# jeffreyyu0602/quantized-training

Hardware: AMD Instinct MI355X
Metric: quantized_elements_per_sec (higher is better)
Workload: dtype bf16; 1 GPU; llama-2-7b-shaped LLaMA (32 layers, hidden 4096, random init) WikiText-style window eval B=1 S=1024 stride 512, fake-quant activation=e4m3 weight=e4m3, --quantize_forward gemm (weights re-quantized every forward); route=eager, parallelism=dp1 (windows round-robin, metric all_gather only), launch=hipGraph replay, valid=True

## Files before the change

### quantized-training_amd/csrc/qt_model_ops.hip

```cpp
#include <hip/hip_runtime.h>
#include <stdint.h>

#include "../../include/qt_hip.h"
#include "qt_device.h"
#include "qt_dispatch.h"
#include "qt_formats.h"
#include "qt_value_codes.h"
#include "qt_value_rows.h"

namespace {

constexpr int kNormThreads = 256;
constexpr int kNormMaxVec = 8;

struct NormExtra {
    uint2 *y8[2];
    qt_format fmt[2];
    int e5m2[2];
};

template <int FQ, bool ADD = false, int EXTRA = 0, int NV = kNormMaxVec>
__global__ __launch_bounds__(kNormThreads) void rmsnorm_kernel(const uint4 *__restrict__ x, const uint4 *__restrict__ w,
                                                               uint4 *__restrict__ y, int nvec, float inv_cols, float eps,
                                                               uint2 *__restrict__ y8, qt_format fmt,
// ... 118 lines not shown
            const float g0 = bf_lo(p[j]), g1 = bf_hi(p[j]);
            const float s0 = bf16_round(g0 / (1.0f + expf(-g0))), s1 = bf16_round(g1 / (1.0f + expf(-g1)));
            pr[j] = pack_bf16x2(s0 * bf_lo(q[j]), s1 * bf_hi(q[j]));
        }
        fq_rows_words<4, false>(pr, o, rnd);
        y[i] = uint4{o[0], o[1], o[2], o[3]};
    }
}

template <bool E5M2>
__global__ __launch_bounds__(256) void silu_mul_fq8_kernel(const uint4 *__restrict__ g, const uint4 *__restrict__ u,
                                                           uint4 *__restrict__ y, uint2 *__restrict__ y8, size_t nvec,
                                                           qt_format fmt, size_t cv, size_t rs_g, size_t rs_u) {
    for (size_t i = (size_t)blockIdx.x * 256 + threadIdx.x; i < nvec; i += (size_t)gridDim.x * 256) {
        const size_t row = i / cv, col = i - row * cv;
        const uint4 a = g[row * rs_g + col], b = u[row * rs_u + col];
        const uint32_t p[4] = {a.x, a.y, a.z, a.w}, q[4] = {b.x, b.y, b.z, b.w};
        uint32_t o[4];
#pragma unroll
        for (int j = 0; j < 4; ++j) {
            const float g0 = bf_lo(p[j]), g1 = bf_hi(p[j]);
            const float s0 = bf16_round(g0 / (1.0f + expf(-g0))), s1 = bf16_round(g1 / (1.0f + expf(-g1)));
            o[j] = pack_bf16x2(s0 * bf_lo(q[j]), s1 * bf_hi(q[j]));
        }
        const uint2 codes = fq8_hw_vec8<E5M2>(o, fmt);
        y[i] = uint4{o[0], o[1], o[2], o[3]};
        y8[i] = codes;
    }
}

struct RopeArgs {
    const uint16_t *x;
    uint16_t *y;
    const uint16_t *cos, *sin;
    long B, S, H, D;
    size_t nvec;
    long rsv;
};

__device__ __forceinline__ void rope_one(const RopeArgs &a, size_t i) {
    const long dv = a.D / 8;
    const long d8 = (long)(i % dv);
    const size_t bsh = i / dv;
    const size_t bs = bsh / (size_t)a.H;
    const long half = dv / 2;
    const bool low = d8 < half;
    const size_t in_row = bs * (size_t)a.rsv + (bsh % (size_t)a.H) * dv;
    const uint4 xv = *(const uint4 *)(a.x + (in_row + d8) * 8);
    const uint4 pv = *(const uint4 *)(a.x + (in_row + (low ? d8 + half : d8 - half)) * 8);
    const uint4 cv = *(const uint4 *)(a.cos + (bs * dv + d8) * 8);
    const uint4 sv = *(const uint4 *)(a.sin + (bs * dv + d8) * 8);
    const uint32_t X[4] = {xv.x, xv.y, xv.z, xv.w}, P[4] = {pv.x, pv.y, pv.z, pv.w};
    const uint32_t C[4] = {cv.x, cv.y, cv.z, cv.w}, S[4] = {sv.x, sv.y, sv.z, sv.w};
    const float sgn = low ? -1.0f : 1.0f;
    uint32_t o[4];
#pragma unroll
    for (int j = 0; j < 4; ++j) {
        const float a0 = bf16_round(bf_lo(X[j]) * bf_lo(C[j])), a1 = bf16_round(bf_hi(X[j]) * bf_hi(C[j]));
        const float b0 = bf16_round(sgn * bf_lo(P[j]) * bf_lo(S[j])), b1 = bf16_round(sgn * bf_hi(P[j]) * bf_hi(S[j]));
        o[j] = pack_bf16x2(a0 + b0, a1 + b1);
    }
    *(uint4 *)(a.y + i * 8) = uint4{o[0], o[1], o[2], o[3]};
}

__global__ __launch_bounds__(256) void rope_kernel(RopeArgs q, RopeArgs k) {
    const size_t total = q.nvec + k.nvec;
    for (size_t i = (size_t)blockIdx.x * 256 + threadIdx.x; i < total; i += (size_t)gridDim.x * 256) {
        if (i < q.nvec) rope_one(q, i);
        else rope_one(k, i - q.nvec);
    }
}

struct RopeFqArgs {
    RopeArgs r;
    qt_format fmt;
    uint8_t *y8;
    int e5m2;
    int inner;
    qt_format inner_fmt;
    const uint16_t *map;
    const uint16_t *rows_lds;
};

template <bool CODES = false>
__device__ __forceinline__ void rope_fq_token(const RopeFqArgs &a, size_t bs0, uint32_t tpb, size_t tokens) {
    const uint32_t dv = (uint32_t)a.r.D / 8, half = dv / 2, nv = (uint32_t)a.r.H * dv;
    const uint32_t S = (uint32_t)a.r.S;
    for (uint32_t i = threadIdx.x; i < tpb * nv; i += 256) {
        const uint32_t lt = tpb == 1 ? 0u : i / nv, v = i - lt * nv;
        const size_t bs = bs0 + lt;
        if (bs >= tokens) break;
        const uint32_t b = (uint32_t)(bs / S), s = (uint32_t)(bs - (size_t)b * S);
        const uint16_t *xrow = a.r.x + bs * (size_t)a.r.rsv * 8;
        const uint16_t *crow = a.r.cos + bs * dv * 8, *srow = a.r.sin + bs * dv * 8;
        const uint32_t h = v / dv, d8 = v - h * dv;
        const bool low = d8 < half;
        const uint4 xv = *(const uint4 *)(xrow + (size_t)v * 8);
        uint32_t out[4] = {xv.x, xv.y, xv.z, xv.w};
        if (a.r.cos) {
            const uint4 pv = *(const uint4 *)(xrow + (size_t)(low ? v + half : v - half) * 8);
            const uint4 cv = *(const uint4 *)(crow + d8 * 8);
            const uint4 sv = *(const uint4 *)(srow + d8 * 8);
            const uint32_t X[4] = {xv.x, xv.y, xv.z, xv.w}, P[4] = {pv.x, pv.y, pv.z, pv.w};
            const uint32_t C[4] = {cv.x, cv.y, cv.z, cv.w}, S[4] = {sv.x, sv.y, sv.z, sv.w};
            const float sgn = low ? -1.0f : 1.0f;
#pragma unroll
            for (int j = 0; j < 4; ++j) {
                float a0 = bf16_round(bf_lo(X[j]) * bf_lo(C[j])), a1 = bf16_round(bf_hi(X[j]) * bf_hi(C[j]));
                if (!CODES && a.inner) {
                    if (a.map) {
                        const Rounder<kFmtRows> rin{a.fmt, a.rows_lds, a.map};
                        a0 = qt_u2f(rin(qt_f2u(a0)));
                        a1 = qt_u2f(rin(qt_f2u(a1)));
                    } else {
                        a0 = qt_u2f(qt_fp_sat_u32(qt_f2u(a0), a.inner_fmt.p0, a.inner_fmt.p1, a.inner_fmt.fhi));
                        a1 = qt_u2f(qt_fp_sat_u32(qt_f2u(a1), a.inner_fmt.p0, a.inner_fmt.p1, a.inner_fmt.fhi));
                    }
                }
                const float b0 = bf16_round(sgn * bf_lo(P[j]) * bf_lo(S[j])), b1 = bf16_round(sgn * bf_hi(P[j]) * bf_hi(S[j]));
                out[j] = pack_bf16x2(a0 + b0, a1 + b1);
            }
        }
        const size_t o = (((size_t)b * (size_t)a.r.H + h) * (size_t)a.r.S + s) * dv + d8;
        if (CODES || a.y8) {
            const uint2 codes = a.e5m2 ? fq8_hw_vec8<true>(out, a.fmt) : fq8_hw_vec8<false>(out, a.fmt);
            *(uint2 *)(a.y8 + o * 8) = codes;
        } else if (a.map) {
            const Rounder<kFmtRows> rnd{a.fmt, a.rows_lds, a.map};
            const uint32_t oin[4] = {out[0], out[1], out[2], out[3]};
            fq_rows_words<4, false>(oin, out, rnd);
        } else {
#pragma unroll
            for (int j = 0; j < 4; ++j) {
                const uint32_t r0 = qt_fp_sat_u32(out[j] << 16, a.fmt.p0, a.fmt.p1, a.fmt.fhi);
                const uint32_t r1 = qt_fp_sat_u32(out[j] & 0xFFFF0000u, a.fmt.p0, a.fmt.p1, a.fmt.fhi);
                out[j] = (r0 >> 16) | (r1 & 0xFFFF0000u);
            }
        }
        if (a.r.y) *(uint4 *)(a.r.y + o * 8) = uint4{out[0], out[1], out[2], out[3]};
    }
}

__global__ __launch_bounds__(256) void rope_fq_kernel(RopeFqArgs q, RopeFqArgs k, unsigned tpb) {
    __shared__ uint4 s_rope_rows[512];
    if (q.map) {
        const uint4 *gr = (const uint4 *)(q.map + QT_MAP_ENTRIES);
        const int nrows = (q.fmt.p1 & 2) ? 512 : 256;
        for (int i = threadIdx.x; i < nrows; i += 256) s_rope_rows[i] = gr[i];
        __syncthreads();
        q.rows_lds = k.rows_lds = (const uint16_t *)s_rope_rows;
    }
    const size_t tokens = (size_t)q.r.B * (size_t)q.r.S;
    for (size_t bs = (size_t)blockIdx.x * tpb; bs < tokens; bs += (size_t)gridDim.x * tpb) {
        rope_fq_token(q, bs, tpb, tokens);
        rope_fq_token(k, bs, tpb, tokens);
    }
}

struct ValueArgs {
    const uint16_t *v;
    uint8_t *vt8;
    long sb, sh, sk, Sk;
    int H, nkb;
    qt_format fmt;
};

template <bool VE5M2, int VD, bool CODES = false>
__global__ __launch_bounds__(256) void rope_fq_value_kernel(RopeFqArgs q, RopeFqArgs k, ValueArgs v, unsigned rope_blocks, unsigned tpb) {
    __shared__ __attribute__((aligned(16))) uint8_t tile[VD * 128];
    if (blockIdx.x < rope_blocks) {
        const size_t tokens = (size_t)q.r.B * (size_t)q.r.S;
        for (size_t bs = (size_t)blockIdx.x * tpb; bs < tokens; bs += (size_t)rope_blocks * tpb) {
            rope_fq_token<CODES>(q, bs, tpb, tokens);
            rope_fq_token<CODES>(k, bs, tpb, tokens);
        }
    } else {
        const unsigned vb = blockIdx.x - rope_blocks;
        value_codes_block<VE5M2, VD>(tile, v.v, v.vt8, (int)(vb % (unsigned)v.nkb), (long)(vb / (unsigned)v.nkb), v.H, v.Sk, v.sb, v.sh, v.sk, v.fmt);
    }
}

struct ValueRowsArgs {
    const uint16_t *v;
    uint16_t *vt;
    long sb, sh, sk, Sk;
    int H, nkb;
};
struct WeightPassArgs {
    const uint4 *w;
    uint4 *wq;
    size_t nvec;
    unsigned blocks;
};

__global__ __launch_bounds__(256) void rope_map_value_kernel(RopeFqArgs q, RopeFqArgs k, ValueRowsArgs v, WeightPassArgs wp, unsigned rope_blocks,
                                                             unsigned tpb) {
    __shared__ __attribute__((aligned(16))) uint16_t tile[value_rows_tile_elems<64>()];
    __shared__ uint4 s_rows[512];
    {
        const uint4 *gr = (const uint4 *)(q.map + QT_MAP_ENTRIES);
        const int nrows = (q.fmt.p1 & 2) ? 512 : 256;
        for (int i = threadIdx.x; i < nrows; i += 256) s_rows[i] = gr[i];
        __syncthreads();
        q.rows_lds = k.rows_lds = (const uint16_t *)s_rows;
    }
    if (blockIdx.x < wp.blocks) {
        const Rounder<kFmtRows> rnd{q.fmt, (const uint16_t *)s_rows, q.map};
        constexpr int kU = 4;
        const size_t stride = (size_t)wp.blocks * 256;
        for (size_t i0 = (size_t)blockIdx.x * 256 + threadIdx.x; i0 < wp.nvec; i0 += stride * kU) {
            uint4 a[kU];
#pragma unroll
            for (int u = 0; u < kU; ++u)
                if (i0 + u * stride < wp.nvec) a[u] = wp.w[i0 + u * stride];
#pragma unroll
            for (int u = 0; u < kU; ++u) {
                if (i0 + u * stride < wp.nvec) {
                    const uint32_t in[4] = {a[u].x, a[u].y, a[u].z, a[u].w};
                    uint32_t o[4];
                    fq_rows_words<4, false>(in, o, rnd);
                    wp.wq[i0 + u * stride] = uint4{o[0], o[1], o[2], o[3]};
                }
            }
        }
        return;
    }
    const unsigned bid = blockIdx.x - wp.blocks;
    if (bid < rope_blocks) {
        const size_t tokens = (size_t)q.r.B * (size_t)q.r.S;
        for (size_t bs = (size_t)bid * tpb; bs < tokens; bs += (size_t)rope_blocks * tpb) {
            rope_fq_token(q, bs, tpb, tokens);
            rope_fq_token(k, bs, tpb, tokens);
        }
    } else {
        const unsigned vb = bid - rope_blocks;
        const Rounder<kFmtRows> rnd{q.fmt, (const uint16_t *)s_rows, q.map};
        value_t_rows_block<64>(tile, rnd, v.v, v.vt, v.H, v.Sk, v.sb, v.sh, v.sk, (long)(vb / (unsigned)v.nkb), (int)(vb % (unsigned)v.nkb), (int)threadIdx.x);
    }
}

struct LnArgs {
    const uint4 *x, *res, *w, *b;
    uint4 *y, *yq;
    uint2 *y8;
    long rows;
    int nvec;
    float inv_cols, eps;
    qt_format fmt;
    int n_extra;
    NormExtra extra;
};

template <int G, int FQ, bool ADD, int NV = kNormMaxVec>
__global__ __launch_bounds__(256) void layernorm_kernel(LnArgs a) {
    constexpr int RPB = 256 / G;
    __shared__ float s_part[2][4];
    const int sub = threadIdx.x / G, lane = threadIdx.x % G;
    const long row = (long)blockIdx.x * RPB + sub;
    if (G == 64 && row >= a.rows) return;
    const size_t base = (size_t)row * (size_t)a.nvec;
    uint4 v[NV];
    float sum = 0.0f;
#pragma unroll
    for (int i = 0; i < NV; ++i) {
        const int c = lane + i * G;
        if (c < a.nvec) {
            v[i] = a.x[base + c];
            if constexpr (ADD) {
                const uint4 r = a.res[base + c];
                v[i].x = pack_bf16x2(bf_lo(v[i].x) + bf_lo(r.x), bf_hi(v[i].x) + bf_hi(r.x));
                v[i].y = pack_bf16x2(bf_lo(v[i].y) + bf_lo(r.y), bf_hi(v[i].y) + bf_hi(r.y));
                v[i].z = pack_bf16x2(bf_lo(v[i].z) + bf_lo(r.z), bf_hi(v[i].z) + bf_hi(r.z));
                v[i].w = pack_bf16x2(bf_lo(v[i].w) + bf_lo(r.w), bf_hi(v[i].w) + bf_hi(r.w));
            }
            sum += (bf_lo(v[i].x) + bf_hi(v[i].x)) + (bf_lo(v[i].y) + bf_hi(v[i].y)) + (bf_lo(v[i].z) + bf_hi(v[i].z)) +
                   (bf_lo(v[i].w) + bf_hi(v[i].w));
        }
    }
    auto reduce = [&](float t, int slot) {
#pragma unroll
        for (int off = 32; off >= 1; off >>= 1) t += __shfl_xor(t, off, 64);
        if constexpr (G == 256) {
            if ((threadIdx.x & 63) == 0) s_part[slot][threadIdx.x >> 6] = t;
            __syncthreads();
            t = (s_part[slot][0] + s_part[slot][1]) + (s_part[slot][2] + s_part[slot][3]);
        }
        return t;
    };
    const float mean = reduce(sum, 0) * a.inv_cols;
    float sq = 0.0f;
#pragma unroll
    for (int i = 0; i < NV; ++i) {
        const int c = lane + i * G;
        if (c < a.nvec) {
            const uint32_t q[4] = {v[i].x, v[i].y, v[i].z, v[i].w};
#pragma unroll
            for (int j = 0; j < 4; ++j) {
                const float d0 = bf_lo(q[j]) - mean, d1 = bf_hi(q[j]) - mean;
                sq += d0 * d0;
                sq += d1 * d1;
            }
        }
    }
    const float rstd = rsqrtf(reduce(sq, 1) * a.inv_cols + a.eps);
#pragma unroll
    for (int i = 0; i < NV; ++i) {
        const int c = lane + i * G;
        if (c < a.nvec) {
            const uint4 ww = a.w[c], bb = a.b[c];
            const uint32_t q[4] = {v[i].x, v[i].y, v[i].z, v[i].w}, g[4] = {ww.x, ww.y, ww.z, ww.w}, h[4] = {bb.x, bb.y, bb.z, bb.w};
            uint32_t o[4];
#pragma unroll
            for (int j = 0; j < 4; ++j)
                o[j] = pack_bf16x2(bf_lo(g[j]) * (rstd * (bf_lo(q[j]) - mean)) + bf_lo(h[j]),
                                   bf_hi(g[j]) * (rstd * (bf_hi(q[j]) - mean)) + bf_hi(h[j]));
// ... 313 lines not shown
}

static int launch_layernorm_any(const LnArgs &a, int fq, bool with_residual, void *stream) {
    hipStream_t st = (hipStream_t)stream;
    const long rows = a.rows;
    const bool residual = with_residual;
    if (a.nvec <= 128) {
        const unsigned blocks = (unsigned)((rows + 3) / 4);
        if (residual) launch_layernorm<64, true>(a, fq, blocks, st);
        else launch_layernorm<64, false>(a, fq, blocks, st);
    } else {
        if (residual) launch_layernorm<256, true>(a, fq, (unsigned)rows, st);
        else launch_layernorm<256, false>(a, fq, (unsigned)rows, st);
    }
    return qt_launch_status();
}

int qt_gelu_bf16(const uint16_t *x, uint16_t *y, uint8_t *y8, size_t n, const qt_format *fmt, void *stream) {
    if (n == 0) return QT_OK;
    if (!x || (!y && !y8)) return QT_ERR_BAD_ARG;
    const int fq = y8 ? qt_fp8_code(fmt) : 0;
    if (y8 && !fq) return QT_ERR_BAD_ARG;
    if ((n & 7) || (((uintptr_t)x | (uintptr_t)y) & 15u) || ((uintptr_t)y8 & 7u)) return QT_ERR_UNALIGNED;
    const size_t nvec = n / 8;
    size_t blocks = (nvec + 255) / 256;
    if (blocks > 256 * 32) blocks = 256 * 32;
    hipStream_t st = (hipStream_t)stream;
    const qt_format f = fq ? *fmt : qt_format{};
    qt_pick<0, 1, 2>(fq, [&](auto FQ) {
        gelu_kernel<decltype(FQ)::value><<<(unsigned)blocks, 256, 0, st>>>((const uint4 *)x, (uint4 *)y, (uint2 *)y8, nvec, f);
    });
    return qt_launch_status();
}

int qt_silu_mul_bf16(const uint16_t *gate, const uint16_t *up, uint16_t *y, size_t rows, size_t cols, size_t gate_row_stride,
                     size_t up_row_stride, void *stream) {
    const size_t n = rows * cols;
    if (n == 0) return QT_OK;
    if (!gate || !up || !y || gate_row_stride < cols || up_row_stride < cols) return QT_ERR_BAD_ARG;
    if ((cols & 7) || ((gate_row_stride | up_row_stride) & 7) || (((uintptr_t)gate | (uintptr_t)up | (uintptr_t)y) & 15u))
        return QT_ERR_UNALIGNED;
    const size_t nvec = n / 8;
    size_t blocks = (nvec + 255) / 256;
    if (blocks > 256 * 32) blocks = 256 * 32;
    silu_mul_kernel<<<(unsigned)blocks, 256, 0, (hipStream_t)stream>>>((const uint4 *)gate, (const uint4 *)up, (uint4 *)y, nvec,
                                                                       cols / 8, gate_row_stride / 8, up_row_stride / 8);
    return qt_launch_status();
}

int qt_silu_mul_fq8_bf16(const uint16_t *gate, const uint16_t *up, uint16_t *y, uint8_t *y8, size_t rows, size_t cols,
                         size_t gate_row_stride, size_t up_row_stride, const qt_format *fmt, void *stream) {
    const size_t n = rows * cols;
    if (n == 0) return QT_OK;
    const int f8 = qt_fp8_code(fmt);
    if (!gate || !up || !y || !y8 || !f8 || gate_row_stride < cols || up_row_stride < cols) return QT_ERR_BAD_ARG;
    if ((cols & 7) || ((gate_row_stride | up_row_stride) & 7) || (((uintptr_t)gate | (uintptr_t)up | (uintptr_t)y) & 15u) ||
        ((uintptr_t)y8 & 7u))
        return QT_ERR_UNALIGNED;
    const size_t nvec = n / 8;
    size_t blocks = (nvec + 255) / 256;
    if (blocks > 256 * 32) blocks = 256 * 32;
    qt_pick_bool(f8 == 2, [&](auto E5M2) {
        silu_mul_fq8_kernel<decltype(E5M2)::value><<<(unsigned)blocks, 256, 0, (hipStream_t)stream>>>((const uint4 *)gate, (const uint4 *)up, (uint4 *)y, (uint2 *)y8, nvec,
                                                                                                      *fmt, cols / 8, gate_row_stride / 8, up_row_stride / 8);
    });
    return qt_launch_status();
}

int qt_rope_bf16(const uint16_t *q, const uint16_t *k, const uint16_t *cos, const uint16_t *sin, uint16_t *q_out,
                 uint16_t *k_out, long B, long S, long Hq, long Hk, long D, long q_row_stride, long k_row_stride, void *stream) {
    if (B * S * D == 0) return QT_OK;
    if (!q || !k || !cos || !sin || !q_out || !k_out || B < 0 || S < 0 || Hq < 0 || Hk < 0) return QT_ERR_BAD_ARG;
    if (D % 16 || (((uintptr_t)q | (uintptr_t)k | (uintptr_t)cos | (uintptr_t)sin | (uintptr_t)q_out | (uintptr_t)k_out) & 15u))
        return QT_ERR_UNALIGNED;
    if (q_row_stride < Hq * D || k_row_stride < Hk * D || (q_row_stride | k_row_stride) % 8) return QT_ERR_BAD_ARG;
    RopeArgs aq{q, q_out, cos, sin, B, S, Hq, D, (size_t)(B * S * Hq * D / 8), q_row_stride / 8};
    RopeArgs ak{k, k_out, cos, sin, B, S, Hk, D, (size_t)(B * S * Hk * D / 8), k_row_stride / 8};
    size_t blocks = (aq.nvec + ak.nvec + 255) / 256;
    if (blocks > 256 * 32) blocks = 256 * 32;
    rope_kernel<<<(unsigned)blocks, 256, 0, (hipStream_t)stream>>>(aq, ak);
    return qt_launch_status();
}

static int rope_fq_launch(const uint16_t *q, const uint16_t *k, const uint16_t *cos, const uint16_t *sin, uint16_t *q_out, uint16_t *k_out,
                          uint8_t *q_out8, uint8_t *k_out8, long B, long S, long Hq, long Hk, long D, long q_row_stride, long k_row_stride,
                          const qt_format *fmt_q, const qt_format *fmt_k, bool need_values, const uint16_t *v, uint8_t *vt8, long v_sb, long v_sh,
                          long v_sk, const qt_format *fmt_v, void *stream, const qt_format *inner_q = nullptr, const qt_format *inner_k = nullptr) {
    if (B * S * D == 0) return QT_OK;
    if ((inner_q && inner_q->kind != QT_FMT_FP_SAT) || (inner_k && inner_k->kind != QT_FMT_FP_SAT) || ((inner_q || inner_k) && !cos)) return QT_ERR_BAD_ARG;
    if (!q || !k || (need_values && !cos) || (cos == nullptr) != (sin == nullptr) || !fmt_q || !fmt_k || B < 0 || S < 0 || Hq < 0 || Hk < 0)
        return QT_ERR_BAD_ARG;
    if (need_values ? (!q_out || !k_out) : (!q_out8 || !k_out8 || (q_out == nullptr) != (k_out == nullptr))) return QT_ERR_BAD_ARG;
    if (fmt_q->kind != QT_FMT_FP_SAT || fmt_k->kind != QT_FMT_FP_SAT) return QT_ERR_BAD_ARG;
    if (D % 16 || (((uintptr_t)q | (uintptr_t)k | (uintptr_t)cos | (uintptr_t)sin | (uintptr_t)q_out | (uintptr_t)k_out) & 15u))
        return QT_ERR_UNALIGNED;
    if (q_row_stride < Hq * D || k_row_stride < Hk * D || (q_row_stride | k_row_stride) % 8) return QT_ERR_BAD_ARG;
    if (((uintptr_t)q_out8 | (uintptr_t)k_out8) & 7u) return QT_ERR_UNALIGNED;
    if ((q_out8 && !qt_fp8_code(fmt_q)) || (k_out8 && !qt_fp8_code(fmt_k))) return QT_ERR_BAD_ARG;
    RopeFqArgs aq{{q, q_out, cos, sin, B, S, Hq, D, (size_t)(B * S * Hq * D / 8), q_row_stride / 8}, *fmt_q, q_out8, qt_fp8_code(fmt_q) == 2 ? 1 : 0,
                  inner_q ? 1 : 0, inner_q ? *inner_q : qt_format{}, nullptr, nullptr};
    RopeFqArgs ak{{k, k_out, cos, sin, B, S, Hk, D, (size_t)(B * S * Hk * D / 8), k_row_stride / 8}, *fmt_k, k_out8, qt_fp8_code(fmt_k) == 2 ? 1 : 0,
                  inner_k ? 1 : 0, inner_k ? *inner_k : qt_format{}, nullptr, nullptr};
    if (Hq * D / 8 > 0xFFFFFFFFl || Hk * D / 8 > 0xFFFFFFFFl || B > 0x7FFFFFFFl || S > 0x7FFFFFFFl) return QT_ERR_BAD_ARG;
    const long nv_max = (Hq > Hk ? Hq : Hk) * D / 8;
    const unsigned tpb = nv_max >= 256 || nv_max < 1 ? 1u : (unsigned)(256 / nv_max);
    size_t blocks = ((size_t)B * (size_t)S + tpb - 1) / tpb;
    if (blocks > 256 * 64) blocks = 256 * 64;
    hipStream_t st = (hipStream_t)stream;
    if (!v) {
        rope_fq_kernel<<<(unsigned)blocks, 256, 0, st>>>(aq, ak, tpb);
        return qt_launch_status();
    }
    if (!vt8 || !qt_fp8_code(fmt_v) || (D != 64 && D != 128) || S % 128 != 0 || B * Hk > 65535) return QT_ERR_BAD_ARG;
    if ((((uintptr_t)v | (uintptr_t)vt8) & 15u) || ((v_sb | v_sh | v_sk) & 7)) return QT_ERR_UNALIGNED;
    ValueArgs av{v, vt8, v_sb, v_sh, v_sk, S, (int)Hk, (int)(S / 128), *fmt_v};
    const unsigned total = (unsigned)blocks + (unsigned)(B * Hk * (S / 128));
    const bool ve5 = qt_fp8_code(fmt_v) == 2;
    if (D == 128) {
        const bool codes = aq.y8 && ak.y8 && !aq.inner && !ak.inner && !aq.map && !ak.map;
        if (codes && !ve5) rope_fq_value_kernel<false, 128, true><<<total, 256, 0, st>>>(aq, ak, av, (unsigned)blocks, tpb);
        else if (ve5) rope_fq_value_kernel<true, 128><<<total, 256, 0, st>>>(aq, ak, av, (unsigned)blocks, tpb);
        else rope_fq_value_kernel<false, 128><<<total, 256, 0, st>>>(aq, ak, av, (unsigned)blocks, tpb);
    } else {
        const bool codes = aq.y8 && ak.y8 && !aq.inner && !ak.inner && !aq.map && !ak.map;
        if (codes && !ve5) rope_fq_value_kernel<false, 64, true><<<total, 256, 0, st>>>(aq, ak, av, (unsigned)blocks, tpb);
        else if (ve5) rope_fq_value_kernel<true, 64><<<total, 256, 0, st>>>(aq, ak, av, (unsigned)blocks, tpb);
        else rope_fq_value_kernel<false, 64><<<total, 256, 0, st>>>(aq, ak, av, (unsigned)blocks, tpb);
    }
    return qt_launch_status();
}

int qt_rope_fq_bf16(const uint16_t *q, const uint16_t *k, const uint16_t *cos, const uint16_t *sin, uint16_t *q_out,
                    uint16_t *k_out, uint8_t *q_out8, uint8_t *k_out8, long B, long S, long Hq, long Hk, long D,
                    long q_row_stride, long k_row_stride, const qt_format *fmt_q, const qt_format *fmt_k, void *stream) {
    return rope_fq_launch(q, k, cos, sin, q_out, k_out, q_out8, k_out8, B, S, Hq, Hk, D, q_row_stride, k_row_stride, fmt_q, fmt_k, true, nullptr,
                          nullptr, 0, 0, 0, nullptr, stream);
}

int qt_rope_fq_value(const uint16_t *q, const uint16_t *k, const uint16_t *cos, const uint16_t *sin, uint16_t *q_out, uint16_t *k_out,
                     uint8_t *q_out8, uint8_t *k_out8, long B, long S, long Hq, long Hk, long D, long q_row_stride, long k_row_stride,
                     const qt_format *fmt_q, const qt_format *fmt_k, const uint16_t *v, uint8_t *vt8, long v_stride_b, long v_stride_h,
                     long v_stride_k, const qt_format *fmt_v, void *stream) {
    return rope_fq_launch(q, k, cos, sin, q_out, k_out, q_out8, k_out8, B, S, Hq, Hk, D, q_row_stride, k_row_stride, fmt_q, fmt_k, false, v, vt8,
                          v_stride_b, v_stride_h, v_stride_k, fmt_v, stream);
}

static bool map_format_ok(const qt_format *fmt, const uint16_t *map) {
    return fmt && map && fmt->kind == QT_FMT_LUT && (fmt->p1 & 1) && (((uintptr_t)map) & 15u) == 0;
}

int qt_rmsnorm_map_bf16(const uint16_t *x, const uint16_t *residual, const uint16_t *weight, uint16_t *sum, uint16_t *y, long rows, long cols,
                        float eps, const qt_format *fmt, const uint16_t *map, int quantize_sum, void *stream) {
    if (rows * cols == 0) return QT_OK;
    if (!x || !weight || !y || rows < 0 || cols < 0 || (residual != nullptr) != (sum != nullptr) || !map_format_ok(fmt, map)) return QT_ERR_BAD_ARG;
    if (cols % 8 || cols > (long)kNormThreads * kNormMaxVec * 8 ||
        (((uintptr_t)x | (uintptr_t)residual | (uintptr_t)weight | (uintptr_t)sum | (uintptr_t)y) & 15u))
        return QT_ERR_UNALIGNED;
    hipStream_t st = (hipStream_t)stream;
    const int nvec = (int)(cols / 8);
    const float inv = 1.0f / (float)cols;
    if (residual) launch_rms<3, true, 0>((unsigned)rows, nvec, st, (const uint4 *)x, (const uint4 *)weight, (uint4 *)y, nvec, inv, eps, nullptr, *fmt, (const uint4 *)residual, (uint4 *)sum, NormExtra{}, quantize_sum ? 3 : 0, qt_format{}, map);
    else launch_rms<3, false, 0>((unsigned)rows, nvec, st, (const uint4 *)x, (const uint4 *)weight, (uint4 *)y, nvec, inv, eps, nullptr, *fmt, nullptr, nullptr, NormExtra{}, 0, qt_format{}, map);
    return qt_launch_status();
}

int qt_silu_mul_map_bf16(const uint16_t *gate, const uint16_t *up, uint16_t *y, size_t rows, size_t cols, size_t gate_row_stride,
                         size_t up_row_stride, const qt_format *fmt, const uint16_t *map, void *stream) {
    if (rows * cols == 0) return QT_OK;
    if (!gate || !up || !y || !map_format_ok(fmt, map)) return QT_ERR_BAD_ARG;
    if (cols % 8 || gate_row_stride % 8 || up_row_stride % 8 || gate_row_stride < cols || up_row_stride < cols ||
        (((uintptr_t)gate | (uintptr_t)up | (uintptr_t)y) & 15u))
        return QT_ERR_UNALIGNED;
    const size_t nvec = rows * cols / 8;
    size_t blocks = (nvec + 255) / 256;
    if (blocks > 256 * 32) blocks = 256 * 32;
    silu_mul_map_kernel<<<(unsigned)blocks, 256, 0, (hipStream_t)stream>>>((const uint4 *)gate, (const uint4 *)up, (uint4 *)y, nvec, *fmt, map, cols / 8,
                                                                          gate_row_stride / 8, up_row_stride / 8);
    return qt_launch_status();
}

int qt_rope_map_bf16(const uint16_t *q, const uint16_t *k, const uint16_t *cos, const uint16_t *sin, uint16_t *q_out, uint16_t *k_out, long B,
                     long S, long Hq, long Hk, long D, long q_row_stride, long k_row_stride, const qt_format *fmt, const uint16_t *map,
                     int inner_q, int inner_k, void *stream) {
    if (B * S * D == 0) return QT_OK;
    if (!q || !k || !cos || !sin || !q_out || !k_out || B < 0 || S < 0 || Hq < 0 || Hk < 0 || !map_format_ok(fmt, map)) return QT_ERR_BAD_ARG;
    if (D % 16 || (((uintptr_t)q | (uintptr_t)k | (uintptr_t)cos | (uintptr_t)sin | (uintptr_t)q_out | (uintptr_t)k_out) & 15u))
        return QT_ERR_UNALIGNED;
    if (q_row_stride < Hq * D || k_row_stride < Hk * D || (q_row_stride | k_row_stride) % 8) return QT_ERR_BAD_ARG;
    if (Hq * D / 8 > 0xFFFFFFFFl || Hk * D / 8 > 0xFFFFFFFFl || B > 0x7FFFFFFFl || S > 0x7FFFFFFFl) return QT_ERR_BAD_ARG;
    RopeFqArgs aq{{q, q_out, cos, sin, B, S, Hq, D, (size_t)(B * S * Hq * D / 8), q_row_stride / 8}, *fmt, nullptr, 0, inner_q ? 1 : 0, qt_format{}, map, nullptr};
    RopeFqArgs ak{{k, k_out, cos, sin, B, S, Hk, D, (size_t)(B * S * Hk * D / 8), k_row_stride / 8}, *fmt, nullptr, 0, inner_k ? 1 : 0, qt_format{}, map, nullptr};
    const long nv_max = (Hq > Hk ? Hq : Hk) * D / 8;
    const unsigned tpb = nv_max >= 256 || nv_max < 1 ? 1u : (unsigned)(256 / nv_max);
    size_t blocks = ((size_t)B * (size_t)S + tpb - 1) / tpb;
    if (blocks > 256 * 64) blocks = 256 * 64;
    rope_fq_kernel<<<(unsigned)blocks, 256, 0, (hipStream_t)stream>>>(aq, ak, tpb);
    return qt_launch_status();
}

static int rope_map_value_launch(const uint16_t *q, const uint16_t *k, const uint16_t *cos, const uint16_t *sin, uint16_t *q_out, uint16_t *k_out,
                                 long B, long S, long Hq, long Hk, long D, long q_row_stride, long k_row_stride, const qt_format *fmt,
                                 const uint16_t *map, int inner_q, int inner_k, const uint16_t *v, uint16_t *vt, long v_stride_b, long v_stride_h,
                                 long v_stride_k, const uint16_t *w, uint16_t *wq, size_t w_elems, void *stream) {
    if (B * S * D == 0) return QT_OK;
    if (!q || !k || !cos || !sin || !q_out || !k_out || !v || !vt || B < 0 || S < 0 || Hq < 0 || Hk < 1 || !map_format_ok(fmt, map)) return QT_ERR_BAD_ARG;
    if (D != kValueRowsD || S % 128 != 0 || B * Hk > 65535 || (w_elems != 0 && (!w || !wq))) return QT_ERR_BAD_ARG;
    if ((((uintptr_t)q | (uintptr_t)k | (uintptr_t)cos | (uintptr_t)sin | (uintptr_t)q_out | (uintptr_t)k_out | (uintptr_t)v | (uintptr_t)vt) & 15u) ||
        ((v_stride_b | v_stride_h | v_stride_k) & 7) || (w_elems != 0 && ((((uintptr_t)w | (uintptr_t)wq) & 15u) || (w_elems & 7))))
        return QT_ERR_UNALIGNED;
    if (q_row_stride < Hq * D || k_row_stride < Hk * D || (q_row_stride | k_row_stride) % 8) return QT_ERR_BAD_ARG;
    if (Hq * D / 8 > 0xFFFFFFFFl || Hk * D / 8 > 0xFFFFFFFFl || B > 0x7FFFFFFFl || S > 0x7FFFFFFFl) return QT_ERR_BAD_ARG;
    RopeFqArgs aq{{q, q_out, cos, sin, B, S, Hq, D, (size_t)(B * S * Hq * D / 8), q_row_stride / 8}, *fmt, nullptr, 0, inner_q ? 1 : 0, qt_format{}, map, nullptr};
    RopeFqArgs ak{{k, k_out, cos, sin, B, S, Hk, D, (size_t)(B * S * Hk * D / 8), k_row_stride / 8}, *fmt, nullptr, 0, inner_k ? 1 : 0, qt_format{}, map, nullptr};
    const long nv_max = (Hq > Hk ? Hq : Hk) * D / 8;
    const unsigned tpb = nv_max >= 256 || nv_max < 1 ? 1u : (unsigned)(256 / nv_max);
    size_t blocks = ((size_t)B * (size_t)S + tpb - 1) / tpb;
    if (blocks > 256 * 64) blocks = 256 * 64;
    ValueRowsArgs av{v, vt, v_stride_b, v_stride_h, v_stride_k, S, (int)Hk, (int)(S / 64)};
    WeightPassArgs aw{(const uint4 *)w, (uint4 *)wq, w_elems / 8, 0};
    if (aw.nvec) {
        size_t wb = (aw.nvec + 256 * 4 - 1) / (256 * 4);
        if (wb > 256 * 2) wb = 256 * 2;
        aw.blocks = (unsigned)wb;
    }
    const unsigned total = aw.blocks + (unsigned)blocks + (unsigned)(B * Hk * (S / 64));
    rope_map_value_kernel<<<total, 256, 0, (hipStream_t)stream>>>(aq, ak, av, aw, (unsigned)blocks, tpb);
    return qt_launch_status();
}

int qt_rope_map_value(const uint16_t *q, const uint16_t *k, const uint16_t *cos, const uint16_t *sin, uint16_t *q_out, uint16_t *k_out, long B,
                      long S, long Hq, long Hk, long D, long q_row_stride, long k_row_stride, const qt_format *fmt, const uint16_t *map,
                      int inner_q, int inner_k, const uint16_t *v, uint16_t *vt, long v_stride_b, long v_stride_h, long v_stride_k, void *stream) {
    return rope_map_value_launch(q, k, cos, sin, q_out, k_out, B, S, Hq, Hk, D, q_row_stride, k_row_stride, fmt, map, inner_q, inner_k, v, vt,
                                 v_stride_b, v_stride_h, v_stride_k, nullptr, nullptr, 0, stream);
}

int qt_rope_map_value_weight(const uint16_t *q, const uint16_t *k, const uint16_t *cos, const uint16_t *sin, uint16_t *q_out, uint16_t *k_out, long B,
                             long S, long Hq, long Hk, long D, long q_row_stride, long k_row_stride, const qt_format *fmt, const uint16_t *map,
                             int inner_q, int inner_k, const uint16_t *v, uint16_t *vt, long v_stride_b, long v_stride_h, long v_stride_k,
                             const uint16_t *w, uint16_t *wq, size_t w_elems, void *stream) {
    return rope_map_value_launch(q, k, cos, sin, q_out, k_out, B, S, Hq, Hk, D, q_row_stride, k_row_stride, fmt, map, inner_q, inner_k, v, vt,
                                 v_stride_b, v_stride_h, v_stride_k, w, wq, w_elems, stream);
}

int qt_rope_fq_inner_value(const uint16_t *q, const uint16_t *k, const uint16_t *cos, const uint16_t *sin, uint16_t *q_out, uint16_t *k_out,
                           uint8_t *q_out8, uint8_t *k_out8, long B, long S, long Hq, long Hk, long D, long q_row_stride, long k_row_stride,
                           const qt_format *fmt_q, const qt_format *fmt_k, const qt_format *inner_q, const qt_format *inner_k, const uint16_t *v,
                           uint8_t *vt8, long v_stride_b, long v_stride_h, long v_stride_k, const qt_format *fmt_v, void *stream) {
    return rope_fq_launch(q, k, cos, sin, q_out, k_out, q_out8, k_out8, B, S, Hq, Hk, D, q_row_stride, k_row_stride, fmt_q, fmt_k, false, v, vt8,
                          v_stride_b, v_stride_h, v_stride_k, fmt_v, stream, inner_q, inner_k);
}

int qt_causal_lm_loss_bf16(const uint16_t *logits, const long long *labels, long batch, long seq_len, long vocab, long row_stride,
                           long long ignore_index, float *row_loss_scratch, float *loss_out, void *stream) {
    if (!logits || !labels || !row_loss_scratch || !loss_out || batch < 1 || seq_len < 1 || vocab < 1 || row_stride < vocab) return QT_ERR_BAD_ARG;
    if (((uintptr_t)logits & 15u) || (row_stride & 7)) return QT_ERR_UNALIGNED;
    const long rows = batch * seq_len;
    if (rows > 0x7FFFFFFFl) return QT_ERR_BAD_ARG;
    hipStream_t st = (hipStream_t)stream;
    nll_rows_kernel<<<(unsigned)rows, 256, 0, st>>>(logits, labels, seq_len, vocab, row_stride, ignore_index, row_loss_scratch);
    nll_mean_kernel<<<1, 256, 0, st>>>(row_loss_scratch, rows, loss_out);
    return qt_launch_status();
}

int qt_colsum_bf16(const uint16_t *x_dev, uint16_t *out_dev, long rows, long cols, void *stream) {
    if (rows < 0 || cols < 0) return QT_ERR_BAD_ARG;
    if (cols == 0) return QT_OK;
    if (!x_dev || !out_dev || cols % 8 != 0) return QT_ERR_BAD_ARG;
    if ((uintptr_t)x_dev & 15u) return QT_ERR_UNALIGNED;
    colsum_kernel<<<(unsigned)((cols + 31) / 32), 256, 0, (hipStream_t)stream>>>(x_dev, out_dev, rows, cols);
    return qt_launch_status();
}

}
```

### quantized-training_amd/csrc/qt_value_codes.h

```cpp
#pragma once
#include "qt_device.h"

namespace {

template <bool E5M2, int D>
__device__ __forceinline__ void value_codes_block(uint8_t *tile , const uint16_t *v, uint8_t *vt8, int kb, long bh, int H,
                                                  long Sk, long sb, long sh, long sk, const qt_format &fmt) {
    const int t = threadIdx.x;
    const long b = bh / H, h = bh % H;
#pragma unroll
    for (int it = 0; it < D / 16; ++it) {
        const int vi = it * 256 + t, key = vi / (D / 8), dv = vi % (D / 8);
        const uint4 in = *(const uint4 *)(v + b * sb + h * sh + ((long)kb * 128 + key) * sk + dv * 8);
        uint32_t o[4] = {in.x, in.y, in.z, in.w};
        const uint2 codes = fq8_hw_vec8<E5M2>(o, fmt);
        const int p = (key & 64) | (((key >> 2) & 3) << 4) | (((key >> 4) & 3) << 2) | (key & 3);
#pragma unroll
        for (int j = 0; j < 8; ++j) tile[(dv * 8 + j) * 128 + p] = (uint8_t)((j < 4 ? codes.x >> (8 * j) : codes.y >> (8 * (j - 4))) & 0xFFu);
    }
    __syncthreads();
#pragma unroll
    for (int it = 0; it < D / 32; ++it) {
        const int ci = it * 256 + t, d = ci >> 3, ch = ci & 7;
        *(uint4 *)(vt8 + (bh * D + d) * Sk + (long)kb * 128 + ch * 16) = *(const uint4 *)(tile + d * 128 + ch * 16);
    }
}

}
```

Before: 883.0 billion elements/s.

## Pair RoPE halves per thread, share cos/sin across Q/K, transpose value codes in registers

The RoPE kernels now give each thread both rotation halves of a head vector and handle Q and K in one pass. Each x/cos/sin vector is loaded once instead of twice, and the cos/sin loads are shared between Q and K. The value-code transpose now gathers four keys per thread and transposes bytes in registers with perm instructions. It writes 32-bit words into an XOR-swizzled LDS tile instead of single bytes, which cuts LDS store count and bank conflicts. A tuning-only env hook for tokens-per-block and value-block ordering is added, and the tokens-per-block formula changes to match the halved work items.

```diff
diff --git a/quantized-training_amd/csrc/qt_model_ops.hip b/quantized-training_amd/csrc/qt_model_ops.hip
--- a/quantized-training_amd/csrc/qt_model_ops.hip
+++ b/quantized-training_amd/csrc/qt_model_ops.hip
@@ -224,62 +224,92 @@
     const uint16_t *rows_lds;
 };
 
+
+template <bool CODES>
+__device__ __forceinline__ void rope_fq_vector(const RopeFqArgs &a, const uint4 &xv, const uint4 &pv, const uint4 &cv, const uint4 &sv, float sgn,
+                                               size_t o) {
+    uint32_t out[4] = {xv.x, xv.y, xv.z, xv.w};
+    if (a.r.cos) {
+        const uint32_t X[4] = {xv.x, xv.y, xv.z, xv.w}, P[4] = {pv.x, pv.y, pv.z, pv.w};
+        const uint32_t C[4] = {cv.x, cv.y, cv.z, cv.w}, S[4] = {sv.x, sv.y, sv.z, sv.w};
+#pragma unroll
+        for (int j = 0; j < 4; ++j) {
+            float a0 = bf16_round(bf_lo(X[j]) * bf_lo(C[j])), a1 = bf16_round(bf_hi(X[j]) * bf_hi(C[j]));
+            if (!CODES && a.inner) {
+                if (a.map) {
+                    const Rounder<kFmtRows> rin{a.fmt, a.rows_lds, a.map};
+                    a0 = qt_u2f(rin(qt_f2u(a0)));
+                    a1 = qt_u2f(rin(qt_f2u(a1)));
+                } else {
+                    a0 = qt_u2f(qt_fp_sat_u32(qt_f2u(a0), a.inner_fmt.p0, a.inner_fmt.p1, a.inner_fmt.fhi));
+                    a1 = qt_u2f(qt_fp_sat_u32(qt_f2u(a1), a.inner_fmt.p0, a.inner_fmt.p1, a.inner_fmt.fhi));
+                }
+            }
+            const float b0 = bf16_round(sgn * bf_lo(P[j]) * bf_lo(S[j])), b1 = bf16_round(sgn * bf_hi(P[j]) * bf_hi(S[j]));
+            out[j] = pack_bf16x2(a0 + b0, a1 + b1);
+        }
+    }
+    if (CODES || a.y8) {
+        const uint2 codes = a.e5m2 ? fq8_hw_vec8<true>(out, a.fmt) : fq8_hw_vec8<false>(out, a.fmt);
+        *(uint2 *)(a.y8 + o * 8) = codes;
+    } else if (a.map) {
+        const Rounder<kFmtRows> rnd{a.fmt, a.rows_lds, a.map};
+        const uint32_t oin[4] = {out[0], out[1], out[2], out[3]};
+        fq_rows_words<4, false>(oin, out, rnd);
+    } else {
+#pragma unroll
+        for (int j = 0; j < 4; ++j) {
+            const uint32_t r0 = qt_fp_sat_u32(out[j] << 16, a.fmt.p0, a.fmt.p1, a.fmt.fhi);
+            const uint32_t r1 = qt_fp_sat_u32(out[j] & 0xFFFF0000u, a.fmt.p0, a.fmt.p1, a.fmt.fhi);
+            out[j] = (r0 >> 16) | (r1 & 0xFFFF0000u);
+        }
+    }
+    if (a.r.y) *(uint4 *)(a.r.y + o * 8) = uint4{out[0], out[1], out[2], out[3]};
+}
+
 template <bool CODES = false>
-__device__ __forceinline__ void rope_fq_token(const RopeFqArgs &a, size_t bs0, uint32_t tpb, size_t tokens) {
-    const uint32_t dv = (uint32_t)a.r.D / 8, half = dv / 2, nv = (uint32_t)a.r.H * dv;
-    const uint32_t S = (uint32_t)a.r.S;
-    for (uint32_t i = threadIdx.x; i < tpb * nv; i += 256) {
-        const uint32_t lt = tpb == 1 ? 0u : i / nv, v = i - lt * nv;
+__device__ __forceinline__ void rope_fq_tokens(const RopeFqArgs &q, const RopeFqArgs &k, size_t bs0, uint32_t tpb, size_t tokens) {
+    const uint32_t dv = (uint32_t)q.r.D / 8, half = dv / 2;
+    const uint32_t npq = (uint32_t)q.r.H * half, npk = (uint32_t)k.r.H * half, np = npq > npk ? npq : npk;
+    const uint32_t S = (uint32_t)q.r.S;
+    float neg = -1.0f, pos = 1.0f;
+    asm("" : "+v"(neg), "+v"(pos));
+    for (uint32_t i = threadIdx.x; i < tpb * np; i += 256) {
+        const uint32_t lt = tpb == 1 ? 0u : i / np, p = i - lt * np;
         const size_t bs = bs0 + lt;
         if (bs >= tokens) break;
         const uint32_t b = (uint32_t)(bs / S), s = (uint32_t)(bs - (size_t)b * S);
-        const uint16_t *xrow = a.r.x + bs * (size_t)a.r.rsv * 8;
-        const uint16_t *crow = a.r.cos + bs * dv * 8, *srow = a.r.sin + bs * dv * 8;
-        const uint32_t h = v / dv, d8 = v - h * dv;
-        const bool low = d8 < half;
-        const uint4 xv = *(const uint4 *)(xrow + (size_t)v * 8);
-        uint32_t out[4] = {xv.x, xv.y, xv.z, xv.w};
-        if (a.r.cos) {
-            const uint4 pv = *(const uint4 *)(xrow + (size_t)(low ? v + half : v - half) * 8);
-            const uint4 cv = *(const uint4 *)(crow + d8 * 8);
-            const uint4 sv = *(const uint4 *)(srow + d8 * 8);
-            const uint32_t X[4] = {xv.x, xv.y, xv.z, xv.w}, P[4] = {pv.x, pv.y, pv.z, pv.w};
-            const uint32_t C[4] = {cv.x, cv.y, cv.z, cv.w}, S[4] = {sv.x, sv.y, sv.z, sv.w};
-            const float sgn = low ? -1.0f : 1.0f;
-#pragma unroll
-            for (int j = 0; j < 4; ++j) {
-                float a0 = bf16_round(bf_lo(X[j]) * bf_lo(C[j])), a1 = bf16_round(bf_hi(X[j]) * bf_hi(C[j]));
-                if (!CODES && a.inner) {
-                    if (a.map) {
-                        const Rounder<kFmtRows> rin{a.fmt, a.rows_lds, a.map};
-                        a0 = qt_u2f(rin(qt_f2u(a0)));
-                        a1 = qt_u2f(rin(qt_f2u(a1)));
-                    } else {
-                        a0 = qt_u2f(qt_fp_sat_u32(qt_f2u(a0), a.inner_fmt.p0, a.inner_fmt.p1, a.inner_fmt.fhi));
-                        a1 = qt_u2f(qt_fp_sat_u32(qt_f2u(a1), a.inner_fmt.p0, a.inner_fmt.p1, a.inner_fmt.fhi));
-                    }
-                }
-                const float b0 = bf16_round(sgn * bf_lo(P[j]) * bf_lo(S[j])), b1 = bf16_round(sgn * bf_hi(P[j]) * bf_hi(S[j]));
-                out[j] = pack_bf16x2(a0 + b0, a1 + b1);
-            }
-        }
-        const size_t o = (((size_t)b * (size_t)a.r.H + h) * (size_t)a.r.S + s) * dv + d8;
-        if (CODES || a.y8) {
-            const uint2 codes = a.e5m2 ? fq8_hw_vec8<true>(out, a.fmt) : fq8_hw_vec8<false>(out, a.fmt);
-            *(uint2 *)(a.y8 + o * 8) = codes;
-        } else if (a.map) {
-            const Rounder<kFmtRows> rnd{a.fmt, a.rows_lds, a.map};
-            const uint32_t oin[4] = {out[0], out[1], out[2], out[3]};
-            fq_rows_words<4, false>(oin, out, rnd);
-        } else {
-#pragma unroll
-            for (int j = 0; j < 4; ++j) {
-                const uint32_t r0 = qt_fp_sat_u32(out[j] << 16, a.fmt.p0, a.fmt.p1, a.fmt.fhi);
-                const uint32_t r1 = qt_fp_sat_u32(out[j] & 0xFFFF0000u, a.fmt.p0, a.fmt.p1, a.fmt.fhi);
-                out[j] = (r0 >> 16) | (r1 & 0xFFFF0000u);
-            }
-        }
-        if (a.r.y) *(uint4 *)(a.r.y + o * 8) = uint4{out[0], out[1], out[2], out[3]};
+        const uint32_t h = p / half, d8 = p - h * half, v = h * dv + d8;
+        const bool in_q = p < npq, in_k = p < npk;
+        const uint4 zero = uint4{0u, 0u, 0u, 0u};
+        uint4 xq[2] = {zero, zero}, xk[2] = {zero, zero}, cs[4] = {zero, zero, zero, zero};
+        if (in_q) {
+            const uint16_t *xrow = q.r.x + bs * (size_t)q.r.rsv * 8;
+            xq[0] = *(const uint4 *)(xrow + (size_t)v * 8);
+            xq[1] = *(const uint4 *)(xrow + (size_t)(v + half) * 8);
+        }
+        if (in_k) {
+            const uint16_t *xrow = k.r.x + bs * (size_t)k.r.rsv * 8;
+            xk[0] = *(const uint4 *)(xrow + (size_t)v * 8);
+            xk[1] = *(const uint4 *)(xrow + (size_t)(v + half) * 8);
+        }
+        if (q.r.cos) {
+            const uint16_t *crow = q.r.cos + bs * dv * 8, *srow = q.r.sin + bs * dv * 8;
+            cs[0] = *(const uint4 *)(crow + d8 * 8);
+            cs[1] = *(const uint4 *)(crow + (d8 + half) * 8);
+            cs[2] = *(const uint4 *)(srow + d8 * 8);
+            cs[3] = *(const uint4 *)(srow + (d8 + half) * 8);
+        }
+        if (in_q) {
+            const size_t o = (((size_t)b * (size_t)q.r.H + h) * (size_t)q.r.S + s) * dv + d8;
+            rope_fq_vector<CODES>(q, xq[0], xq[1], cs[0], cs[2], neg, o);
+            rope_fq_vector<CODES>(q, xq[1], xq[0], cs[1], cs[3], pos, o + half);
+        }
+        if (in_k) {
+            const size_t o = (((size_t)b * (size_t)k.r.H + h) * (size_t)k.r.S + s) * dv + d8;
+            rope_fq_vector<CODES>(k, xk[0], xk[1], cs[0], cs[2], neg, o);
+            rope_fq_vector<CODES>(k, xk[1], xk[0], cs[1], cs[3], pos, o + half);
+        }
     }
 }
 
@@ -294,8 +324,7 @@
     }
     const size_t tokens = (size_t)q.r.B * (size_t)q.r.S;
     for (size_t bs = (size_t)blockIdx.x * tpb; bs < tokens; bs += (size_t)gridDim.x * tpb) {
-        rope_fq_token(q, bs, tpb, tokens);
-        rope_fq_token(k, bs, tpb, tokens);
+        rope_fq_tokens(q, k, bs, tpb, tokens);
     }
 }
 
@@ -308,16 +337,16 @@
 };
 
 template <bool VE5M2, int VD, bool CODES = false>
-__global__ __launch_bounds__(256) void rope_fq_value_kernel(RopeFqArgs q, RopeFqArgs k, ValueArgs v, unsigned rope_blocks, unsigned tpb) {
+__global__ __launch_bounds__(256) void rope_fq_value_kernel(RopeFqArgs q, RopeFqArgs k, ValueArgs v, unsigned rope_blocks, unsigned tpb,
+                                                            unsigned value_first) {
     __shared__ __attribute__((aligned(16))) uint8_t tile[VD * 128];
-    if (blockIdx.x < rope_blocks) {
+    const unsigned value_blocks = gridDim.x - rope_blocks;
+    const unsigned rb = value_first ? blockIdx.x - value_blocks : blockIdx.x;
+    if (rb < rope_blocks) {
         const size_t tokens = (size_t)q.r.B * (size_t)q.r.S;
-        for (size_t bs = (size_t)blockIdx.x * tpb; bs < tokens; bs += (size_t)rope_blocks * tpb) {
-            rope_fq_token<CODES>(q, bs, tpb, tokens);
-            rope_fq_token<CODES>(k, bs, tpb, tokens);
-        }
+        for (size_t bs = (size_t)rb * tpb; bs < tokens; bs += (size_t)rope_blocks * tpb) rope_fq_tokens<CODES>(q, k, bs, tpb, tokens);
     } else {
-        const unsigned vb = blockIdx.x - rope_blocks;
+        const unsigned vb = value_first ? blockIdx.x : blockIdx.x - rope_blocks;
         value_codes_block<VE5M2, VD>(tile, v.v, v.vt8, (int)(vb % (unsigned)v.nkb), (long)(vb / (unsigned)v.nkb), v.H, v.Sk, v.sb, v.sh, v.sk, v.fmt);
     }
 }
@@ -371,8 +400,7 @@
     if (bid < rope_blocks) {
         const size_t tokens = (size_t)q.r.B * (size_t)q.r.S;
         for (size_t bs = (size_t)bid * tpb; bs < tokens; bs += (size_t)rope_blocks * tpb) {
-            rope_fq_token(q, bs, tpb, tokens);
-            rope_fq_token(k, bs, tpb, tokens);
+            rope_fq_tokens(q, k, bs, tpb, tokens);
         }
     } else {
         const unsigned vb = bid - rope_blocks;
@@ -852,6 +880,11 @@
     return qt_launch_status();
 }
 
+static unsigned rope_tokens_per_block(long Hq, long Hk, long D) {
+    const long np_max = (Hq > Hk ? Hq : Hk) * D / 16;
+    return np_max >= 256 || np_max < 1 ? 1u : (unsigned)(256 / np_max);
+}
+
 static int rope_fq_launch(const uint16_t *q, const uint16_t *k, const uint16_t *cos, const uint16_t *sin, uint16_t *q_out, uint16_t *k_out,
                           uint8_t *q_out8, uint8_t *k_out8, long B, long S, long Hq, long Hk, long D, long q_row_stride, long k_row_stride,
                           const qt_format *fmt_q, const qt_format *fmt_k, bool need_values, const uint16_t *v, uint8_t *vt8, long v_sb, long v_sh,
@@ -872,8 +905,12 @@
     RopeFqArgs ak{{k, k_out, cos, sin, B, S, Hk, D, (size_t)(B * S * Hk * D / 8), k_row_stride / 8}, *fmt_k, k_out8, qt_fp8_code(fmt_k) == 2 ? 1 : 0,
                   inner_k ? 1 : 0, inner_k ? *inner_k : qt_format{}, nullptr, nullptr};
     if (Hq * D / 8 > 0xFFFFFFFFl || Hk * D / 8 > 0xFFFFFFFFl || B > 0x7FFFFFFFl || S > 0x7FFFFFFFl) return QT_ERR_BAD_ARG;
-    const long nv_max = (Hq > Hk ? Hq : Hk) * D / 8;
-    const unsigned tpb = nv_max >= 256 || nv_max < 1 ? 1u : (unsigned)(256 / nv_max);
+    unsigned tpb = rope_tokens_per_block(Hq, Hk, D);
+    unsigned value_first = 0;
+#ifdef QT_TUNING_BUILD
+    if (const char *e = getenv("QT_ROPE_TPB")) tpb = (unsigned)atoi(e) > 0 ? (unsigned)atoi(e) : tpb;
+    if (const char *e = getenv("QT_ROPE_VALUE_FIRST")) value_first = atoi(e) != 0;
+#endif
     size_t blocks = ((size_t)B * (size_t)S + tpb - 1) / tpb;
     if (blocks > 256 * 64) blocks = 256 * 64;
     hipStream_t st = (hipStream_t)stream;
@@ -888,14 +925,14 @@
     const bool ve5 = qt_fp8_code(fmt_v) == 2;
     if (D == 128) {
         const bool codes = aq.y8 && ak.y8 && !aq.inner && !ak.inner && !aq.map && !ak.map;
-        if (codes && !ve5) rope_fq_value_kernel<false, 128, true><<<total, 256, 0, st>>>(aq, ak, av, (unsigned)blocks, tpb);
-        else if (ve5) rope_fq_value_kernel<true, 128><<<total, 256, 0, st>>>(aq, ak, av, (unsigned)blocks, tpb);
-        else rope_fq_value_kernel<false, 128><<<total, 256, 0, st>>>(aq, ak, av, (unsigned)blocks, tpb);
+        if (codes && !ve5) rope_fq_value_kernel<false, 128, true><<<total, 256, 0, st>>>(aq, ak, av, (unsigned)blocks, tpb, value_first);
+        else if (ve5) rope_fq_value_kernel<true, 128><<<total, 256, 0, st>>>(aq, ak, av, (unsigned)blocks, tpb, value_first);
+        else rope_fq_value_kernel<false, 128><<<total, 256, 0, st>>>(aq, ak, av, (unsigned)blocks, tpb, value_first);
     } else {
         const bool codes = aq.y8 && ak.y8 && !aq.inner && !ak.inner && !aq.map && !ak.map;
-        if (codes && !ve5) rope_fq_value_kernel<false, 64, true><<<total, 256, 0, st>>>(aq, ak, av, (unsigned)blocks, tpb);
-        else if (ve5) rope_fq_value_kernel<true, 64><<<total, 256, 0, st>>>(aq, ak, av, (unsigned)blocks, tpb);
-        else rope_fq_value_kernel<false, 64><<<total, 256, 0, st>>>(aq, ak, av, (unsigned)blocks, tpb);
+        if (codes && !ve5) rope_fq_value_kernel<false, 64, true><<<total, 256, 0, st>>>(aq, ak, av, (unsigned)blocks, tpb, value_first);
+        else if (ve5) rope_fq_value_kernel<true, 64><<<total, 256, 0, st>>>(aq, ak, av, (unsigned)blocks, tpb, value_first);
+        else rope_fq_value_kernel<false, 64><<<total, 256, 0, st>>>(aq, ak, av, (unsigned)blocks, tpb, value_first);
     }
     return qt_launch_status();
 }
@@ -960,8 +997,7 @@
     if (Hq * D / 8 > 0xFFFFFFFFl || Hk * D / 8 > 0xFFFFFFFFl || B > 0x7FFFFFFFl || S > 0x7FFFFFFFl) return QT_ERR_BAD_ARG;
     RopeFqArgs aq{{q, q_out, cos, sin, B, S, Hq, D, (size_t)(B * S * Hq * D / 8), q_row_stride / 8}, *fmt, nullptr, 0, inner_q ? 1 : 0, qt_format{}, map, nullptr};
     RopeFqArgs ak{{k, k_out, cos, sin, B, S, Hk, D, (size_t)(B * S * Hk * D / 8), k_row_stride / 8}, *fmt, nullptr, 0, inner_k ? 1 : 0, qt_format{}, map, nullptr};
-    const long nv_max = (Hq > Hk ? Hq : Hk) * D / 8;
-    const unsigned tpb = nv_max >= 256 || nv_max < 1 ? 1u : (unsigned)(256 / nv_max);
+    const unsigned tpb = rope_tokens_per_block(Hq, Hk, D);
     size_t blocks = ((size_t)B * (size_t)S + tpb - 1) / tpb;
     if (blocks > 256 * 64) blocks = 256 * 64;
     rope_fq_kernel<<<(unsigned)blocks, 256, 0, (hipStream_t)stream>>>(aq, ak, tpb);
@@ -982,8 +1018,7 @@
     if (Hq * D / 8 > 0xFFFFFFFFl || Hk * D / 8 > 0xFFFFFFFFl || B > 0x7FFFFFFFl || S > 0x7FFFFFFFl) return QT_ERR_BAD_ARG;
     RopeFqArgs aq{{q, q_out, cos, sin, B, S, Hq, D, (size_t)(B * S * Hq * D / 8), q_row_stride / 8}, *fmt, nullptr, 0, inner_q ? 1 : 0, qt_format{}, map, nullptr};
     RopeFqArgs ak{{k, k_out, cos, sin, B, S, Hk, D, (size_t)(B * S * Hk * D / 8), k_row_stride / 8}, *fmt, nullptr, 0, inner_k ? 1 : 0, qt_format{}, map, nullptr};
-    const long nv_max = (Hq > Hk ? Hq : Hk) * D / 8;
-    const unsigned tpb = nv_max >= 256 || nv_max < 1 ? 1u : (unsigned)(256 / nv_max);
+    const unsigned tpb = rope_tokens_per_block(Hq, Hk, D);
     size_t blocks = ((size_t)B * (size_t)S + tpb - 1) / tpb;
     if (blocks > 256 * 64) blocks = 256 * 64;
     ValueRowsArgs av{v, vt, v_stride_b, v_stride_h, v_stride_k, S, (int)Hk, (int)(S / 64)};
diff --git a/quantized-training_amd/csrc/qt_value_codes.h b/quantized-training_amd/csrc/qt_value_codes.h
--- a/quantized-training_amd/csrc/qt_value_codes.h
+++ b/quantized-training_amd/csrc/qt_value_codes.h
@@ -2,27 +2,48 @@
 #include "qt_device.h"
 
 namespace {
+
+__device__ __forceinline__ void transpose_4x4_bytes(uint32_t a, uint32_t b, uint32_t c, uint32_t d, uint32_t *w) {
+    const uint32_t ab_lo = __builtin_amdgcn_perm(b, a, 0x05010400u), ab_hi = __builtin_amdgcn_perm(b, a, 0x07030602u);
+    const uint32_t cd_lo = __builtin_amdgcn_perm(d, c, 0x05010400u), cd_hi = __builtin_amdgcn_perm(d, c, 0x07030602u);
+    w[0] = __builtin_amdgcn_perm(cd_lo, ab_lo, 0x05040100u);
+    w[1] = __builtin_amdgcn_perm(cd_lo, ab_lo, 0x07060302u);
+    w[2] = __builtin_amdgcn_perm(cd_hi, ab_hi, 0x05040100u);
+    w[3] = __builtin_amdgcn_perm(cd_hi, ab_hi, 0x07060302u);
+}
 
 template <bool E5M2, int D>
 __device__ __forceinline__ void value_codes_block(uint8_t *tile , const uint16_t *v, uint8_t *vt8, int kb, long bh, int H,
                                                   long Sk, long sb, long sh, long sk, const qt_format &fmt) {
     const int t = threadIdx.x;
     const long b = bh / H, h = bh % H;
+    const uint16_t *vblk = v + b * sb + h * sh + (long)kb * 128 * sk;
+    uint32_t *tile32 = (uint32_t *)tile;
 #pragma unroll
-    for (int it = 0; it < D / 16; ++it) {
-        const int vi = it * 256 + t, key = vi / (D / 8), dv = vi % (D / 8);
-        const uint4 in = *(const uint4 *)(v + b * sb + h * sh + ((long)kb * 128 + key) * sk + dv * 8);
-        uint32_t o[4] = {in.x, in.y, in.z, in.w};
-        const uint2 codes = fq8_hw_vec8<E5M2>(o, fmt);
-        const int p = (key & 64) | (((key >> 2) & 3) << 4) | (((key >> 4) & 3) << 2) | (key & 3);
+    for (int it = 0; it < D / 64; ++it) {
+        const int u = (it * 256 + t) >> 5, l = t & 31;
+        const int dv = (l & 7) | ((u >> 3) << 3), kg = (u & 3) | ((l >> 3) << 2) | (((u >> 2) & 1) << 4);
+        uint2 codes[4];
+        uint4 in[4];
 #pragma unroll
-        for (int j = 0; j < 8; ++j) tile[(dv * 8 + j) * 128 + p] = (uint8_t)((j < 4 ? codes.x >> (8 * j) : codes.y >> (8 * (j - 4))) & 0xFFu);
+        for (int r = 0; r < 4; ++r) in[r] = *(const uint4 *)(vblk + (long)(kg * 4 + r) * sk + dv * 8);
+#pragma unroll
+        for (int r = 0; r < 4; ++r) {
+            uint32_t o[4] = {in[r].x, in[r].y, in[r].z, in[r].w};
+            codes[r] = fq8_hw_vec8<E5M2>(o, fmt);
+        }
+        const int chunk = (((kg >> 4) << 2) | (kg & 3)) ^ (dv & 7), word = (kg >> 2) & 3;
+        uint32_t w[8];
+        transpose_4x4_bytes(codes[0].x, codes[1].x, codes[2].x, codes[3].x, w);
+        transpose_4x4_bytes(codes[0].y, codes[1].y, codes[2].y, codes[3].y, w + 4);
+#pragma unroll
+        for (int j = 0; j < 8; ++j) tile32[(dv * 8 + j) * 32 + chunk * 4 + word] = w[j];
     }
     __syncthreads();
 #pragma unroll
     for (int it = 0; it < D / 32; ++it) {
         const int ci = it * 256 + t, d = ci >> 3, ch = ci & 7;
-        *(uint4 *)(vt8 + (bh * D + d) * Sk + (long)kb * 128 + ch * 16) = *(const uint4 *)(tile + d * 128 + ch * 16);
+        *(uint4 *)(vt8 + (bh * D + d) * Sk + (long)kb * 128 + ch * 16) = *(const uint4 *)(tile + d * 128 + ((ch ^ ((d >> 3) & 7)) << 4));
     }
 }
 
```

New measurement: 879.1 billion elements/s. Within noise of the previous version (-0.4%).
